# xvyaward/qeft

Measured on AMD Instinct MI355X. Metric: decode tokens/sec, Llama-2-7B w4 g128 r128, higher is better.
Workload: dtype f16; 1 GPU; llama-2-7b w4 g128 r128 full decode step, batch 1, greedy, KV context 69..1248 tokens (64-token context + 5 warm-up tokens before the timed region); layers=32, hipgraph=True, parallelism=single GPU

## Files before the change

### qeft_amd/csrc/decode_attn.h

```cpp
#pragma once
#include "qeft_common.h"

namespace qeft {

template <int CTRL>
__device__ __forceinline__ float dpp_mov(float v) {
    return __builtin_bit_cast(float, __builtin_amdgcn_update_dpp(0, __builtin_bit_cast(int, v), CTRL, 0xF, 0xF, true));
}
__device__ __forceinline__ float wave_max(float v) {
    v = fmaxf(v, dpp_mov<0xB1>(v));
    v = fmaxf(v, dpp_mov<0x4E>(v));
    v = fmaxf(v, dpp_mov<0x141>(v));
    v = fmaxf(v, dpp_mov<0x140>(v));
    v = fmaxf(v, __shfl_xor(v, 16));
    v = fmaxf(v, __shfl_xor(v, 32));
    return v;
}

__device__ __forceinline__ void st_agent(float* p, float v) { __hip_atomic_store(p, v, __ATOMIC_RELAXED, __HIP_MEMORY_SCOPE_AGENT); }
__device__ __forceinline__ float ld_agent(const float* p) { return __hip_atomic_load(p, __ATOMIC_RELAXED, __HIP_MEMORY_SCOPE_AGENT); }

constexpr int kAttnRec = 132;
__host__ __device__ constexpr size_t attn_ctr_floats(int n_heads) { return ((size_t)n_heads + 3) / 4 * 4; }

template <bool KFT>
__device__ __forceinline__ size_t kcache_off(int p, int chunk, int max_seq) {
    return KFT ? ((size_t)chunk * max_seq + p) * 8 : (size_t)p * 128 + chunk * 8;
}

template <int PRE, int DH = 1, bool KFT = false, bool DBG = false, bool ALIBI = false, bool ROW = true>
__device__ __forceinline__ void rope_attn_decode_body(uint8_t* smem_raw, const int bid, const int* __restrict__ pos_ptr,
                                                      const int* __restrict__ out_pos, const f16* __restrict__ q,
                                                      const f16* __restrict__ k, const f16* __restrict__ v,
                                                      const float* __restrict__ cs, uint32_t heads_kv_s_tab,
                                                      const float* __restrict__ sn, f16* __restrict__ kc, f16* __restrict__ vc,
                                                      f16* __restrict__ out, float* __restrict__ ws, int max_seq,
                                                      unsigned long long* dbg_ptr, const float* __restrict__ alibi,
                                                      f16* __restrict__ pub = nullptr) {
    constexpr int HD = 128;
    const int n_heads = (int)(heads_kv_s_tab & 0xfffu), n_kv = (int)((heads_kv_s_tab >> 12) & 0xfffu);
    const int S = (int)((heads_kv_s_tab >> 24) & 0xfu);
    unsigned long long* const dbg = DBG ? dbg_ptr : nullptr;
    unsigned long long stamp[10];
    auto mark = [&](int i) {
        if (dbg) { __builtin_amdgcn_sched_barrier(0); stamp[i] = __builtin_amdgcn_s_memtime(); __builtin_amdgcn_sched_barrier(0); }
    };
    unsigned long long rt0 = dbg ? __builtin_amdgcn_s_memrealtime() : 0;
    mark(0);
    float* prob = (float*)smem_raw;
    float* part = prob + max_seq + 16;
    float* psum = part + 16 * HD;
    float* wm = psum + 64;
    f16* knew = (f16*)(wm + 4);
    f16* vnew = knew + HD;
    f16* qs = vnew + HD;
    __shared__ int last_ticket;

    constexpr int HDB = HD / DH;
    constexpr int NDG = 16 / DH;
    constexpr int NPC = 64 / NDG;
    constexpr int PPC = 16 / NPC;
    const int dhi = (int)(bid % DH);
    const int hs_idx = bid / DH;
    const int h = hs_idx / S, sp = hs_idx % S, t = threadIdx.x, lane = t & 63;
    const int w = __builtin_amdgcn_readfirstlane(t >> 6);
    const int gw = sp * 4 + w, NW = 4 * S;
    const int grp = n_heads / n_kv, hk = h / grp;
    f16* kch = kc + (size_t)hk * max_seq * HD;
    f16* vch = vc + (size_t)hk * max_seq * HD;
    const bool appender = (sp == 0) && (dhi == 0) && (h % grp == 0);
    const float slope = ALIBI ? alibi[h] : 0.f;

    const int ti = dhi * HDB + (t & (HDB - 1));
    const f16* src = (t < 64) ? q + h * HD + t : (t < 128) ? k + hk * HD + (t - 64) : v + hk * HD + (t - 128);
    const f16 raw_a = src[0];
    const f16 raw_b = src[(t < 128) ? 64 : 0];
    float rc, rsn;
    if constexpr (ROW) {
        rc = cs[t & 63];
        rsn = sn[t & 63];
    }
    int opos_raw = 0;
    if (out_pos) opos_raw = out_pos[h * HD + ti];
    mark(1);
    const int pos = *pos_ptr, L = pos + 1;
    if (pos < 0 || pos >= max_seq) return;
    if (dbg) { asm volatile("" :: "s"(pos)); }
    if constexpr (!ROW) {
        rc = cs[(size_t)pos * 64 + (t & 63)];
        rsn = sn[(size_t)pos * 64 + (t & 63)];
    }
    mark(2);
    const int qd = lane & 3, pj = lane >> 2;
    const int dg = lane & (NDG - 1), pc = lane / NDG;
    const int dim0 = dhi * HDB + dg * 8;
    h8 kpre[PRE][4], vpre[PRE][PPC];
#pragma unroll
    for (int i = 0; i < PRE; ++i) {
        const int r0 = (i * NW + gw) * 16;
        const int krow = r0 < L ? r0 + pj : 0;
#pragma unroll
        for (int j = 0; j < 4; ++j) kpre[i][j] = *(const h8*)(kch + kcache_off<KFT>(krow, qd + 4 * j, max_seq));
    }
#pragma unroll
    for (int i = 0; i < PRE; ++i) {
        const int r0 = (i * NW + gw) * 16;
        const int vrow = r0 < L ? r0 + pc * PPC : 0;
        const h8* row = (const h8*)(vch + (size_t)vrow * HD + dim0);
#pragma unroll
        for (int j = 0; j < PPC; ++j) vpre[i][j] = row[j * (HD / 8)];
    }
    const int opos = out_pos ? opos_raw : h * HD + ti;
    const float ra = (float)raw_a, rb = (float)raw_b;
    const int i = t & 63;
    const float c = rc, sv = rsn;
    float r0 = ra * c - rb * sv, r1 = rb * c + ra * sv;
    asm("" : "+v"(r0), "+v"(r1));
    const float scale = 0.08838834764831845f;
    const f16 q0 = (f16)(r0 * scale), q1 = (f16)(r1 * scale);
    const f16 k0 = (f16)r0, k1 = (f16)r1;
    const f16 vv = (f16)ra;
    {
        f16* const d0 = knew + t + ((t < 64) ? 2 * HD : (t < 128) ? -64 : 0);
        d0[0] = (t < 64) ? q0 : (t < 128) ? k0 : vv;
        d0[(t < 128) ? 64 : 0] = (t < 64) ? q1 : (t < 128) ? k1 : vv;
    }
    if (appender) {
        if (t >= 128) {
            vch[(size_t)pos * HD + (t - 128)] = vv;
        } else if (t >= 64) {
            kch[kcache_off<KFT>(pos, i >> 3, max_seq) + (i & 7)] = k0;
            kch[kcache_off<KFT>(pos, (i >> 3) + 8, max_seq) + (i & 7)] = k1;
        }
    }
    asm volatile("s_waitcnt lgkmcnt(0)\n\ts_barrier" ::: "memory");
    mark(3);

    h2 qreg[16];
#pragma unroll
    for (int j = 0; j < 16; ++j) qreg[j] = *(const h2*)(qs + (j >> 2) * 32 + qd * 8 + 2 * (j & 3));
    float snew = 0.f;
#pragma unroll
    for (int j = 0; j < 16; ++j) snew = dot2(qreg[j], *(const h2*)(knew + (j >> 2) * 32 + qd * 8 + 2 * (j & 3)), snew);
    float lmax = -3.0e38f;
    auto score_run = [&](int i, const h8* kr, bool live) {
        const int p = (i * NW + gw) * 16 + pj;
        float sdot = 0.f;
#pragma unroll
        for (int j = 0; j < 4; ++j) {
            const u32x4 kw = __builtin_bit_cast(u32x4, kr[j]);
#pragma unroll
            for (int e = 0; e < 4; ++e) sdot = dot2(qreg[j * 4 + e], as_h2(kw[e]), sdot);
        }
        sdot = (p == pos) ? snew : sdot;
        sdot += dpp_mov<0xB1>(sdot);
        sdot += dpp_mov<0x4E>(sdot);
        if constexpr (ALIBI) sdot += slope * (float)(p - pos);
        sdot = (p >= L) ? -3.0e38f : sdot;
        if (qd == 0) prob[live ? p : max_seq + pj] = sdot;
        lmax = fmaxf(lmax, sdot);
    };
#pragma unroll
    for (int i = 0; i < PRE; ++i) score_run(i, kpre[i], (i * NW + gw) * 16 < L);
    for (int i = PRE; (i * NW + gw) * 16 < L; ++i) {
        h8 kr[4];
#pragma unroll
        for (int j = 0; j < 4; ++j) kr[j] = *(const h8*)(kch + kcache_off<KFT>((i * NW + gw) * 16 + pj, qd + 4 * j, max_seq));
        score_run(i, kr, true);
    }
    const float mw = wave_max(lmax);
    mark(4);
    __builtin_amdgcn_wave_barrier();

    float o[8];
#pragma unroll
    for (int e = 0; e < 8; ++e) o[e] = 0.f;
    float lsum = 0.f;
    const h8 vn = *(const h8*)(vnew + dim0);
    auto pv_run = [&](int i, const h8* vr, bool live) {
        const int p0 = (i * NW + gw) * 16 + pc * PPC;
        const int s0 = live ? p0 : max_seq + pc * PPC;
        float sraw[PPC];
#pragma unroll
        for (int j = 0; j < PPC; ++j) sraw[j] = prob[s0 + j];
#pragma unroll
        for (int j = 0; j < PPC; ++j) {
            const int p = p0 + j;
            const float ex = __expf(sraw[j] - mw);
            const float e = (p < L) ? ex : 0.f;
            const h8 vv = (p < pos) ? vr[j] : vn;
            lsum += e;
#pragma unroll
            for (int d = 0; d < 8; ++d) o[d] += e * (float)vv[d];
        }
    };
#pragma unroll
    for (int i = 0; i < PRE; ++i) pv_run(i, vpre[i], (i * NW + gw) * 16 < L);
    for (int i = PRE; (i * NW + gw) * 16 < L; ++i) {
        h8 vr[PPC];
#pragma unroll
        for (int j = 0; j < PPC; ++j)
            vr[j] = *(const h8*)(vch + (size_t)((i * NW + gw) * 16 + pc * PPC + j) * HD + dim0);
        pv_run(i, vr, true);
    }
    {
        float* dst = part + (w * NPC + pc) * HDB + dg * 8;
        *(f32x4*)dst = f32x4{o[0], o[1], o[2], o[3]};
        *(f32x4*)(dst + 4) = f32x4{o[4], o[5], o[6], o[7]};
        if (dg == 0) psum[w * NPC + pc] = lsum;
        if (lane == 0) wm[w] = mw;
    }
    mark(5);
    __syncthreads();
    mark(6);
    const float M = fmaxf(fmaxf(wm[0], wm[1]), fmaxf(wm[2], wm[3]));
    float acc = 0.f, den = 0.f;
    if (t < HDB) {
#pragma unroll
        for (int g = 0; g < 4 * NPC; ++g) {
            const float f = __expf(wm[g / NPC] - M);
            acc += f * part[g * HDB + t];
            den += f * psum[g];
        }
    }
    if (S == 1) {
        if (t < HDB) {
            const f16 ov = (f16)(acc / den);
            if (pub) __hip_atomic_store((uint16_t*)pub + opos, __builtin_bit_cast(uint16_t, ov), __ATOMIC_RELAXED, __HIP_MEMORY_SCOPE_AGENT);
            else out[opos] = ov;
        }
        if (dbg && lane == 0) {
            mark(7);
            unsigned long long* d = dbg + ((size_t)bid * 4 + w) * 12;
            d[0] = rt0; d[1] = __builtin_amdgcn_s_memrealtime();
            for (int i = 0; i < 8; ++i) d[2 + i] = stamp[i];
            d[10] = d[11] = 0;
        }
        return;
    }
    float* rec = ws + attn_ctr_floats(n_heads) + (size_t)(h * S + sp) * kAttnRec;
    if (t < HD) st_agent(rec + t, acc);
    if (t == 0) {
        st_agent(rec + HD, M);
        st_agent(rec + HD + 1, den);
    }
    asm volatile("s_waitcnt vmcnt(0)" ::: "memory");
    __syncthreads();
    mark(7);
    unsigned* ctr = (unsigned*)ws + h;
    if (t == 0) {
        const unsigned ticket = __hip_atomic_fetch_add(ctr, 1u, __ATOMIC_RELAXED, __HIP_MEMORY_SCOPE_AGENT);
        last_ticket = (ticket == (unsigned)(S - 1));
        if (ticket == (unsigned)(S - 1)) __hip_atomic_store(ctr, 0u, __ATOMIC_RELAXED, __HIP_MEMORY_SCOPE_AGENT);
    }
    __syncthreads();
    mark(8);
    if (dbg && lane == 0 && !last_ticket) {
        unsigned long long* d = dbg + ((size_t)bid * 4 + w) * 12;
        d[0] = rt0; d[1] = __builtin_amdgcn_s_memrealtime();
        for (int i = 0; i < 9; ++i) d[2 + i] = stamp[i];
        d[11] = 0;
    }
    if (!last_ticket) return;
    if (t < HD) {
        const float* r0 = ws + attn_ctr_floats(n_heads) + (size_t)h * S * kAttnRec;
        float Mh = -3.0e38f;
        for (int j = 0; j < S; ++j) Mh = fmaxf(Mh, ld_agent(r0 + j * kAttnRec + HD));
        float a2 = 0.f, d2 = 0.f;
        for (int j = 0; j < S; ++j) {
            const float f = __expf(ld_agent(r0 + j * kAttnRec + HD) - Mh);
            a2 += f * ld_agent(r0 + j * kAttnRec + t);
            d2 += f * ld_agent(r0 + j * kAttnRec + HD + 1);
        }
        out[opos] = (f16)(a2 / d2);
    }
    if (dbg && lane == 0) {
        mark(9);
        unsigned long long* d = dbg + ((size_t)bid * 4 + w) * 12;
        d[0] = rt0; d[1] = __builtin_amdgcn_s_memrealtime();
        for (int i = 0; i < 9; ++i) d[2 + i] = stamp[i];
        d[11] = stamp[9];
    }
}

template <int PRE, int DH = 1, bool KFT = false, bool DBG = false, bool ALIBI = false, bool ROW = true>
__global__ __launch_bounds__(256) void rope_attn_decode_kernel(const int* __restrict__ pos_ptr, const int* __restrict__ out_pos,
                                                               const f16* __restrict__ q, const f16* __restrict__ k,
                                                               const f16* __restrict__ v, const float* __restrict__ cs,
                                                               uint32_t heads_kv_s_tab, const float* __restrict__ sn,
                                                               f16* __restrict__ kc, f16* __restrict__ vc, f16* __restrict__ out,
                                                               float* __restrict__ ws, int max_seq, unsigned long long* dbg_ptr,
                                                               const float* __restrict__ alibi) {
    extern __shared__ __attribute__((aligned(16))) uint8_t smem_raw[];
    rope_attn_decode_body<PRE, DH, KFT, DBG, ALIBI, ROW>(smem_raw, (int)blockIdx.x, pos_ptr, out_pos, q, k, v, cs, heads_kv_s_tab, sn, kc, vc, out, ws,
                                                    max_seq, dbg_ptr, alibi);
}

__host__ __device__ inline size_t rope_attn_smem_bytes(int max_seq) { return (size_t)(max_seq + 16) * 4 + 16 * 128 * 4 + 64 * 4 + 4 * 4 + 3 * 128 * 2; }

}
```

### qeft_amd/csrc/decode_aux.hip

```cpp
#include <cstdlib>

#include "qeft_common.h"
#include "host_launch.h"
#include "decode_attn.h"

namespace qeft {

__device__ __forceinline__ float block_sum_256(float v, float* sm) {
    v = wave_sum(v);
    const int lane = threadIdx.x & 63, wave = threadIdx.x >> 6;
    __syncthreads();
    if (lane == 0) sm[wave] = v;
    __syncthreads();
    return sm[0] + sm[1] + sm[2] + sm[3];
}

__device__ __forceinline__ float block_max_256(float v, float* sm) {
#pragma unroll
    for (int o = 32; o > 0; o >>= 1) v = fmaxf(v, __shfl_xor(v, o));
    const int lane = threadIdx.x & 63, wave = threadIdx.x >> 6;
    __syncthreads();
    if (lane == 0) sm[wave] = v;
    __syncthreads();
    return fmaxf(fmaxf(sm[0], sm[1]), fmaxf(sm[2], sm[3]));
}

__global__ __launch_bounds__(256) void rmsnorm_kernel(const f16* __restrict__ x, const f16* __restrict__ add,
                                                      const f16* __restrict__ gamma, f16* __restrict__ res_out,
                                                      f16* __restrict__ y, int H, float eps) {
    __shared__ float sm[4];
    const size_t base = (size_t)blockIdx.x * H;
    float ss = 0.f;
    for (int i = threadIdx.x * 8; i < H; i += 256 * 8) {
        h8 v = *(const h8*)(x + base + i);
        if (add) {
            const h8 w = *(const h8*)(add + base + i);
#pragma unroll
            for (int j = 0; j < 8; ++j) v[j] = (f16)((float)v[j] + (float)w[j]);
            if (res_out) *(h8*)(res_out + base + i) = v;
        }
#pragma unroll
        for (int j = 0; j < 8; ++j) ss += (float)v[j] * (float)v[j];
    }
    ss = block_sum_256(ss, sm);
    const float rs = rsqrtf(ss / (float)H + eps);
    for (int i = threadIdx.x * 8; i < H; i += 256 * 8) {
        h8 v = *(const h8*)(x + base + i);
        if (add) {
            const h8 w = *(const h8*)(add + base + i);
#pragma unroll
            for (int j = 0; j < 8; ++j) v[j] = (f16)((float)v[j] + (float)w[j]);
        }
        const h8 g = *(const h8*)(gamma + i);
        h8 o;
#pragma unroll
        for (int j = 0; j < 8; ++j) o[j] = mul_f32_to_f16((float)v[j] * rs, (float)g[j]);
        *(h8*)(y + base + i) = o;
    }
}

__global__ __launch_bounds__(256) void silu_mul_kernel(const f16* __restrict__ gate, const f16* __restrict__ up,
                                                       f16* __restrict__ out, int n) {
    const int i = (blockIdx.x * 256 + threadIdx.x) * 8;
    if (i >= n) return;
    const h8 g = *(const h8*)(gate + i), u = *(const h8*)(up + i);
    h8 o;
#pragma unroll
    for (int j = 0; j < 8; ++j) {
        o[j] = mul_f32_to_f16(silu_f32((float)g[j]), (float)u[j]);
    }
    *(h8*)(out + i) = o;
}

__global__ __launch_bounds__(256) void token_begin_kernel(const f16* __restrict__ embed, const long long* __restrict__ tok,
                                                          const float* __restrict__ rope_tab, const int* __restrict__ pos,
                                                          f16* __restrict__ h, float* __restrict__ rope_row, int hidden,
                                                          int vocab, int max_seq) {
    const long long tk = min(max(*tok, 0ll), (long long)vocab - 1);
    const int i = (blockIdx.x * 256 + threadIdx.x) * 8;
    if (i < hidden) *(h8*)(h + i) = *(const h8*)(embed + (size_t)tk * hidden + i);
    if (blockIdx.x == 0 && threadIdx.x < 128 && rope_row) {
        const int p = min(max(*pos, 0), max_seq - 1);
        rope_row[threadIdx.x] = rope_tab[(size_t)p * 128 + threadIdx.x];
    }
}

__global__ __launch_bounds__(256) void token_begin_norm_kernel(const f16* __restrict__ embed, const long long* __restrict__ tok,
                                                               const float* __restrict__ rope_tab, const int* __restrict__ pos,
                                                               float* __restrict__ h, float* __restrict__ rope_row,
                                                               const f16* __restrict__ gamma, f16* __restrict__ hnorm,
                                                               float* __restrict__ ssq_out, int hidden, int vocab, int max_seq) {
    __shared__ float sm[4];
    const long long tk = min(max(*tok, 0ll), (long long)vocab - 1);
    const int i = (blockIdx.x * 256 + threadIdx.x) * 8;
    float ss = 0.f;
    if (i < hidden) {
        const h8 v = *(const h8*)(embed + (size_t)tk * hidden + i), g = *(const h8*)(gamma + i);
        h8 o;
#pragma unroll
        for (int j = 0; j < 8; ++j) {
            ss += (float)v[j] * (float)v[j];
            o[j] = mul_f32_to_f16((float)v[j], (float)g[j]);
            h[i + j] = (float)v[j];
        }
        *(h8*)(hnorm + i) = o;
    }
    ss = block_sum_256(ss, sm);
    if (threadIdx.x == 0) ssq_out[blockIdx.x] = ss;
    if (blockIdx.x == 0 && threadIdx.x < 128 && rope_row) {
        const int p = min(max(*pos, 0), max_seq - 1);
        rope_row[threadIdx.x] = rope_tab[(size_t)p * 128 + threadIdx.x];
    }
}

__global__ __launch_bounds__(256) void residual_norm_kernel(const float* __restrict__ h, const f16* __restrict__ add,
                                                            const f16* __restrict__ gamma, float* __restrict__ h_out,
                                                            f16* __restrict__ hnorm, float* __restrict__ ssq_out, int hidden) {
    __shared__ float sm[4];
    const int i = (blockIdx.x * 256 + threadIdx.x) * 8;
    float ss = 0.f;
    if (i < hidden) {
        float v[8];
#pragma unroll
        for (int j = 0; j < 8; ++j) v[j] = h[i + j];
        if (add) {
            const h8 w = *(const h8*)(add + i);
#pragma unroll
            for (int j = 0; j < 8; ++j) v[j] += (float)w[j];
        }
#pragma unroll
        for (int j = 0; j < 8; ++j) h_out[i + j] = v[j];
        if (gamma) {
            const h8 g = *(const h8*)(gamma + i);
            h8 o;
#pragma unroll
            for (int j = 0; j < 8; ++j) {
                ss += v[j] * v[j];
                o[j] = mul_f32_to_f16(v[j], (float)g[j]);
            }
            *(h8*)(hnorm + i) = o;
        }
    }
    if (gamma) {
        ss = block_sum_256(ss, sm);
        if (threadIdx.x == 0) ssq_out[blockIdx.x] = ss;
    }
}

__global__ __launch_bounds__(256) void rmsnorm_f32_kernel(const float* __restrict__ x, const f16* __restrict__ gamma,
                                                          f16* __restrict__ y, int H, float eps) {
    __shared__ float sm[4];
    const size_t base = (size_t)blockIdx.x * H;
    float ss = 0.f;
    for (int i = threadIdx.x; i < H; i += 256) ss += x[base + i] * x[base + i];
    ss = block_sum_256(ss, sm);
    const float rs = rsqrtf(ss / (float)H + eps);
    for (int i = threadIdx.x; i < H; i += 256) y[base + i] = mul_f32_to_f16(x[base + i] * rs, (float)gamma[i]);
}

__global__ __launch_bounds__(256) void rope_rows_kernel(f16* __restrict__ x, const float* __restrict__ cs,
                                                        const float* __restrict__ sn, int H, int row_stride) {
    const int t = blockIdx.x, i = threadIdx.x & 63;
    const float c = cs[(size_t)t * 64 + i], s = sn[(size_t)t * 64 + i];
    for (int h = threadIdx.x >> 6; h < H; h += 4) {
        f16* p = x + (size_t)t * row_stride + h * 128;
        const float a = (float)p[i], b = (float)p[i + 64];
        p[i] = (f16)(a * c - b * s);
        p[i + 64] = (f16)(b * c + a * s);
    }
}

hipError_t rope_rows_launch(void* x, const void* cs, const void* sn, int T, int H, int row_stride, hipStream_t st) {
    hipLaunchKernelGGL(rope_rows_kernel, dim3(T), dim3(256), 0, st, (f16*)x, (const float*)cs, (const float*)sn, H, row_stride);
    return hipGetLastError();
}

template <int LPR>
__global__ __launch_bounds__(512) void lm_head_f16_kernel(const float* __restrict__ h32, const f16* __restrict__ gamma,
                                                          const f16* __restrict__ W, f16* __restrict__ logits, int vocab,
                                                          float eps, int rows_per_block) {
    constexpr int H = 512 * LPR;
    __shared__ float red[8];
    const int tid = threadIdx.x, lane = tid & 63;
    const int wave = __builtin_amdgcn_readfirstlane(tid >> 6);
    float xv[LPR][8];
    float ss = 0.f;
#pragma unroll
    for (int c = 0; c < LPR; ++c) {
        const f32x4 a = *(const f32x4*)(h32 + c * 512 + lane * 8), b = *(const f32x4*)(h32 + c * 512 + lane * 8 + 4);
#pragma unroll
        for (int j = 0; j < 4; ++j) {
            xv[c][j] = a[j];
            xv[c][4 + j] = b[j];
            ss += a[j] * a[j] + b[j] * b[j];
        }
    }
    ss = wave_sum(ss);
    const float rs = rsqrtf(ss / (float)H + eps);
    h2 xh[LPR][4];
#pragma unroll
    for (int c = 0; c < LPR; ++c) {
        const h8 g = *(const h8*)(gamma + c * 512 + lane * 8);
#pragma unroll
        for (int j = 0; j < 4; ++j)
            xh[c][j] = h2{mul_f32_to_f16(xv[c][2 * j] * rs, (float)g[2 * j]), mul_f32_to_f16(xv[c][2 * j + 1] * rs, (float)g[2 * j + 1])};
    }
    (void)red;
    const int r_end = min(vocab, (int)(blockIdx.x + 1) * rows_per_block);
    int r = blockIdx.x * rows_per_block + wave;
    u32x4 cur[LPR], nxt[LPR];
    auto load_row = [&](int row, u32x4 (&dst)[LPR]) {
        const u32x4* p = (const u32x4*)(W + (size_t)min(row, vocab - 1) * H) + lane;
#pragma unroll
        for (int c = 0; c < LPR; ++c) dst[c] = __builtin_nontemporal_load(p + c * 64);
    };
    load_row(r, cur);
    for (; r < r_end; r += 8) {
        load_row(r + 8, nxt);
        float acc = 0.f;
#pragma unroll
        for (int c = 0; c < LPR; ++c)
#pragma unroll
            for (int j = 0; j < 4; ++j) acc = __builtin_amdgcn_fdot2(as_h2(cur[c][j]), xh[c][j], acc, false);
        acc = wave_sum(acc);
        if (lane == 0) logits[r] = (f16)acc;
#pragma unroll
        for (int c = 0; c < LPR; ++c) cur[c] = nxt[c];
    }
}

hipError_t lm_head_f16_launch(const void* h32, const void* gamma, const void* W, void* logits, int H, int vocab, float eps,
                              hipStream_t st) {
    const int blocks = vocab >= 4096 ? 512 : (vocab + 7) / 8, rpb = (vocab + blocks - 1) / blocks;
    auto go = [&](auto kern) {
        hipLaunchKernelGGL(kern, dim3(blocks), dim3(512), 0, st, (const float*)h32, (const f16*)gamma, (const f16*)W, (f16*)logits,
                           vocab, eps, rpb);
        return hipGetLastError();
    };
    switch (H) {
        case 512: return go(lm_head_f16_kernel<1>);
        case 1024: return go(lm_head_f16_kernel<2>);
        case 2048: return go(lm_head_f16_kernel<4>);
        case 4096: return go(lm_head_f16_kernel<8>);
        case 5120: return go(lm_head_f16_kernel<10>);
        case 8192: return go(lm_head_f16_kernel<16>);
        default: return hipErrorInvalidValue;
    }
}

__global__ __launch_bounds__(1024) void token_end_kernel(const f16* __restrict__ logits, long long* __restrict__ tok,
                                                         int* __restrict__ pos, int vocab, int greedy) {
    __shared__ float bv[16];
    __shared__ int bi[16];
    const int t = threadIdx.x;
    if (greedy) {
        float best = -INFINITY;
        int idx = 0x7fffffff;
        for (int i = t * 8; i < vocab; i += 1024 * 8) {
            if (i + 8 <= vocab) {
                const h8 v = *(const h8*)(logits + i);
#pragma unroll
                for (int j = 0; j < 8; ++j)
                    if ((float)v[j] > best) { best = (float)v[j]; idx = i + j; }
            } else {
                for (int j = i; j < vocab; ++j)
                    if ((float)logits[j] > best) { best = (float)logits[j]; idx = j; }
            }
        }
#pragma unroll
        for (int o = 32; o > 0; o >>= 1) {
            const float ob = __shfl_xor(best, o);
            const int oi = __shfl_xor(idx, o);
            if (ob > best || (ob == best && oi < idx)) { best = ob; idx = oi; }
        }
        if ((t & 63) == 0) { bv[t >> 6] = best; bi[t >> 6] = idx; }
        __syncthreads();
        if (t == 0) {
            for (int w = 1; w < 16; ++w)
                if (bv[w] > best || (bv[w] == best && bi[w] < idx)) { best = bv[w]; idx = bi[w]; }
            *tok = idx == 0x7fffffff ? 0 : idx;
        }
    }
    if (t == 0) *pos = *pos + 1;
}

hipError_t token_begin_launch(const void* embed, const void* tok, const void* rope_tab, const int* pos, void* h,
                              void* rope_row, int hidden, int vocab, int max_seq, hipStream_t st) {
    hipLaunchKernelGGL(token_begin_kernel, dim3((hidden / 8 + 255) / 256), dim3(256), 0, st, (const f16*)embed,
                       (const long long*)tok, (const float*)rope_tab, pos, (f16*)h, (float*)rope_row, hidden, vocab, max_seq);
    return hipGetLastError();
}

int token_begin_norm_blocks(int hidden) { return (hidden / 8 + 255) / 256; }

hipError_t token_begin_norm_launch(const void* embed, const void* tok, const void* rope_tab, const int* pos, void* h,
                                   void* rope_row, const void* gamma, void* hnorm, float* ssq_out, int hidden, int vocab,
                                   int max_seq, hipStream_t st) {
    hipLaunchKernelGGL(token_begin_norm_kernel, dim3(token_begin_norm_blocks(hidden)), dim3(256), 0, st, (const f16*)embed,
                       (const long long*)tok, (const float*)rope_tab, pos, (float*)h, (float*)rope_row, (const f16*)gamma,
                       (f16*)hnorm, ssq_out, hidden, vocab, max_seq);
    return hipGetLastError();
}

hipError_t residual_norm_launch(const void* h, const void* add, const void* gamma, void* h_out, void* hnorm, float* ssq_out,
                                int hidden, hipStream_t st) {
    hipLaunchKernelGGL(residual_norm_kernel, dim3(token_begin_norm_blocks(hidden)), dim3(256), 0, st, (const float*)h,
                       (const f16*)add, (const f16*)gamma, (float*)h_out, (f16*)hnorm, ssq_out, hidden);
    return hipGetLastError();
}

hipError_t rmsnorm_f32_launch(const void* x, const void* gamma, void* y, int m, int H, float eps, hipStream_t st) {
    hipLaunchKernelGGL(rmsnorm_f32_kernel, dim3(m), dim3(256), 0, st, (const float*)x, (const f16*)gamma, (f16*)y, H, eps);
    return hipGetLastError();
}

hipError_t token_end_launch(const void* logits, void* tok, int* pos, int vocab, int greedy, hipStream_t st) {
    hipLaunchKernelGGL(token_end_kernel, dim3(1), dim3(1024), 0, st, (const f16*)logits, (long long*)tok, pos, vocab, greedy);
    return hipGetLastError();
}

hipError_t rmsnorm_launch(const void* x, const void* add, const void* gamma, void* res_out, void* y, int m, int H,
                          float eps, hipStream_t st) {
    hipLaunchKernelGGL(rmsnorm_kernel, dim3(m), dim3(256), 0, st, (const f16*)x, (const f16*)add, (const f16*)gamma,
                       (f16*)res_out, (f16*)y, H, eps);
    return hipGetLastError();
}

hipError_t silu_mul_launch(const void* gate, const void* up, void* out, int n, hipStream_t st) {
    hipLaunchKernelGGL(silu_mul_kernel, dim3((n / 8 + 255) / 256), dim3(256), 0, st, (const f16*)gate, (const f16*)up,
                       (f16*)out, n);
    return hipGetLastError();
}

unsigned long long* g_attn_dbg = nullptr;
#ifndef QEFT_ATTN_PRE1
#define QEFT_ATTN_PRE1 4
#endif
size_t attn_workspace_bytes(int n_heads, int S) { return S > 1 ? (attn_ctr_floats(n_heads) + (size_t)n_heads * S * kAttnRec) * 4 : 0; }

hipError_t rope_attn_decode_launch(const void* q, const void* k, const void* v, const void* cs, const void* sn, void* kc,
                                   void* vc, const int* pos, const int* out_pos, void* out, void* ws, int n_heads,
                                   int n_kv, int max_seq, int S, int tab_rows, hipStream_t st, bool k_ft_layout,
                                   const float* alibi_slopes) {
    const size_t smem = (size_t)(max_seq + 16) * 4 + 16 * 128 * 4 + 64 * 4 + 4 * 4 + 3 * 128 * 2;
    int dh = 1;
    auto launch = [&](auto kern) -> hipError_t {
        if (smem > 64 * 1024) {
            hipError_t e = hipFuncSetAttribute((const void*)kern, hipFuncAttributeMaxDynamicSharedMemorySize, (int)smem);
            if (e != hipSuccess) return e;
        }
        if (n_heads > 4095 || n_kv > 4095 || S > 15) return hipErrorInvalidValue;
        const uint32_t packed = (uint32_t)n_heads | ((uint32_t)n_kv << 12) | ((uint32_t)S << 24);
        hipLaunchKernelGGL(kern, dim3(n_heads * S * dh), dim3(256), smem, st, pos, out_pos, (const f16*)q, (const f16*)k,
                           (const f16*)v, (const float*)cs, packed, (const float*)sn, (f16*)kc, (f16*)vc, (f16*)out, (float*)ws,
                           max_seq, g_attn_dbg, alibi_slopes);
        return hipGetLastError();
    };
    static const int dh_env = getenv("QEFT_ATTN_DH") ? atoi(getenv("QEFT_ATTN_DH")) : 2;
    const bool row = tab_rows == 1;
#define QEFT_ATTN_FORM(...) (row ? launch(rope_attn_decode_kernel<__VA_ARGS__, true>) : launch(rope_attn_decode_kernel<__VA_ARGS__, false>))
    if (k_ft_layout) {
        if (S != 1) return hipErrorInvalidValue;
        if (alibi_slopes) return QEFT_ATTN_FORM(4, 1, true, false, true);
        return QEFT_ATTN_FORM(4, 1, true, false, false);
    }
    if (g_attn_dbg) {
        if (S == 1 && dh_env == 2) {
            dh = 2;
            return QEFT_ATTN_FORM(4, 2, false, true, false);
        }
        if (S == 1) return QEFT_ATTN_FORM(4, 1, false, true, false);
        if (S == 2) return QEFT_ATTN_FORM(2, 1, false, true, false);
        return QEFT_ATTN_FORM(1, 1, false, true, false);
    }
    if (S == 1 && dh_env == 4) {
        dh = 4;
        return QEFT_ATTN_FORM(QEFT_ATTN_PRE1, 4, false, false, false);
    }
    if (S == 1 && dh_env == 2) {
        dh = 2;
        return QEFT_ATTN_FORM(QEFT_ATTN_PRE1, 2, false, false, false);
    }
    if (S == 1) return QEFT_ATTN_FORM(QEFT_ATTN_PRE1, 1, false, false, false);
    if (S == 2) return QEFT_ATTN_FORM(2, 1, false, false, false);
    return QEFT_ATTN_FORM(1, 1, false, false, false);
#undef QEFT_ATTN_FORM
}

__global__ __launch_bounds__(256) void sqa_generic_kernel(const f16* __restrict__ q, const f16* __restrict__ k, const f16* __restrict__ v,
                                                          f16* __restrict__ kc, f16* __restrict__ vc, const int* __restrict__ pos_ptr,
                                                          const float* __restrict__ alibi, f16* __restrict__ out, int n_heads, int n_kv,
                                                          int max_seq, int D) {
    extern __shared__ __attribute__((aligned(16))) uint8_t smem_raw[];
    float* qs = (float*)smem_raw;
    float* knew = qs + 256;
    float* vnew = knew + 256;
    float* red = vnew + 256;
    float* prob = red + 256;
    const int h = blockIdx.x, t = threadIdx.x;
    const int grp = n_heads / n_kv, hk = h / grp;
    const int pos = *pos_ptr, L = pos + 1;
    if (pos < 0 || pos >= max_seq) return;
    f16* kch = kc + (size_t)hk * max_seq * D;
    f16* vch = vc + (size_t)hk * max_seq * D;
    const float scale = __builtin_amdgcn_rsqf((float)D);
    if (t < D) {
        const f16 kv = k[hk * D + t], vv = v[hk * D + t];
        qs[t] = (float)q[h * D + t] * scale;
        knew[t] = (float)kv;
        vnew[t] = (float)vv;
        if (h % grp == 0) {
            kch[((size_t)(t >> 3) * max_seq + pos) * 8 + (t & 7)] = kv;
            vch[(size_t)pos * D + t] = vv;
        }
    }
    __syncthreads();
    const float slope = alibi ? alibi[h] : 0.f;
    float lmax = -3.0e38f;
    for (int p = t; p < L; p += 256) {
        float sdot = 0.f;
        if (p == pos) {
            for (int d = 0; d < D; ++d) sdot += qs[d] * knew[d];
        } else {
            for (int c = 0; c < D / 8; ++c) {
                const h8 kk = *(const h8*)(kch + ((size_t)c * max_seq + p) * 8);
#pragma unroll
                for (int e = 0; e < 8; ++e) sdot += qs[c * 8 + e] * (float)kk[e];
            }
        }
        sdot += slope * (float)(p - pos);
        prob[p] = sdot;
        lmax = fmaxf(lmax, sdot);
    }
    red[t] = lmax;
    __syncthreads();
    for (int s = 128; s > 0; s >>= 1) {
        if (t < s) red[t] = fmaxf(red[t], red[t + s]);
        __syncthreads();
    }
    const float m = red[0];
    __syncthreads();
    float lsum = 0.f;
    for (int p = t; p < L; p += 256) {
        const float e = __expf(prob[p] - m);
        prob[p] = e;
        lsum += e;
    }
    red[t] = lsum;
    __syncthreads();
    for (int s = 128; s > 0; s >>= 1) {
        if (t < s) red[t] += red[t + s];
        __syncthreads();
    }
    const float inv = 1.f / red[0];
    __syncthreads();
    const int NG = 256 / D > 0 ? 256 / D : 1;
    float o = 0.f;
    const int d = t % D, pcl = t / D;
    if (pcl < NG)
        for (int p = pcl; p < L; p += NG) o += prob[p] * (p == pos ? vnew[d] : (float)vch[(size_t)p * D + d]);
    red[t] = pcl < NG ? o : 0.f;
    __syncthreads();
    if (t < D) {
        float acc = 0.f;
        for (int g = 0; g < NG; ++g) acc += red[g * D + t];
        out[h * D + t] = (f16)(acc * inv);
    }
}

hipError_t sqa_generic_launch(const void* q, const void* k, const void* v, void* kc, void* vc, const int* pos, const float* alibi,
                              void* out, int n_heads, int n_kv, int max_seq, int head_dim, hipStream_t st) {
    const size_t smem = (size_t)(4 * 256 + max_seq) * 4;
    if (smem > 64 * 1024) {
        const hipError_t e = hipFuncSetAttribute((const void*)sqa_generic_kernel, hipFuncAttributeMaxDynamicSharedMemorySize, (int)smem);
        if (e != hipSuccess) return e;
    }
    hipLaunchKernelGGL(sqa_generic_kernel, dim3(n_heads), dim3(256), smem, st, (const f16*)q, (const f16*)k, (const f16*)v, (f16*)kc, (f16*)vc,
                       pos, alibi, (f16*)out, n_heads, n_kv, max_seq, head_dim);
    return hipGetLastError();
}

}
```

Measured before the change: 766.8 tokens/s.

## Prefetch early KV cache rows before reading decode position in attention

Issues the first EARLY K (and possibly V) cache loads before the dependent load of the position pointer, so the cache fetches overlap that load instead of waiting behind it. The rows loaded early are bounded by max_seq rather than the live length. Kernel arguments are repacked into a geometry word with a power-of-two group shift, log2 of the split count and max_seq/16, which replaces integer divisions. A new table form reads sin from the cos table when the two are contiguous. The early loads may fetch rows beyond the live context, costing some extra bandwidth, and the split count is now limited to powers of two up to 8.

```diff
diff --git a/qeft_amd/csrc/decode_attn.h b/qeft_amd/csrc/decode_attn.h
--- a/qeft_amd/csrc/decode_attn.h
+++ b/qeft_amd/csrc/decode_attn.h
@@ -28,18 +28,20 @@
     return KFT ? ((size_t)chunk * max_seq + p) * 8 : (size_t)p * 128 + chunk * 8;
 }
 
-template <int PRE, int DH = 1, bool KFT = false, bool DBG = false, bool ALIBI = false, bool ROW = true>
-__device__ __forceinline__ void rope_attn_decode_body(uint8_t* smem_raw, const int bid, const int* __restrict__ pos_ptr,
-                                                      const int* __restrict__ out_pos, const f16* __restrict__ q,
+template <int PRE, int DH = 1, bool KFT = false, bool DBG = false, bool ALIBI = false, int ROW = 1, int EARLY_ = 0>
+__device__ __forceinline__ void rope_attn_decode_body(uint8_t* smem_raw, const int bid, const f16* __restrict__ q,
                                                       const f16* __restrict__ k, const f16* __restrict__ v,
-                                                      const float* __restrict__ cs, uint32_t heads_kv_s_tab,
-                                                      const float* __restrict__ sn, f16* __restrict__ kc, f16* __restrict__ vc,
-                                                      f16* __restrict__ out, float* __restrict__ ws, int max_seq,
+                                                      const float* __restrict__ cs, const int* __restrict__ out_pos,
+                                                      f16* __restrict__ kc, uint32_t geom, int n_heads, f16* __restrict__ vc,
+                                                      const float* __restrict__ sn, const int* __restrict__ pos_ptr,
+                                                      f16* __restrict__ out, float* __restrict__ ws,
                                                       unsigned long long* dbg_ptr, const float* __restrict__ alibi,
                                                       f16* __restrict__ pub = nullptr) {
     constexpr int HD = 128;
-    const int n_heads = (int)(heads_kv_s_tab & 0xfffu), n_kv = (int)((heads_kv_s_tab >> 12) & 0xfffu);
-    const int S = (int)((heads_kv_s_tab >> 24) & 0xfu);
+    constexpr int EARLY = ROW == 0 ? 0 : EARLY_ < PRE ? EARLY_ : PRE;
+    const int grp = (int)(geom & 0xfffu), gsh = (int)((geom >> 12) & 0xfu);
+    const int lgS = DH > 1 ? 0 : (int)((geom >> 16) & 3u), S = 1 << lgS;
+    const int max_seq = (int)((geom >> 18) & 0xfffu) * 16;
     unsigned long long* const dbg = DBG ? dbg_ptr : nullptr;
     unsigned long long stamp[10];
     auto mark = [&](int i) {
@@ -60,15 +62,14 @@
     constexpr int NDG = 16 / DH;
     constexpr int NPC = 64 / NDG;
     constexpr int PPC = 16 / NPC;
-    const int dhi = (int)(bid % DH);
-    const int hs_idx = bid / DH;
-    const int h = hs_idx / S, sp = hs_idx % S, t = threadIdx.x, lane = t & 63;
+    const int dhi = (int)((unsigned)bid % DH);
+    const int hs_idx = (int)((unsigned)bid / DH);
+    const int h = hs_idx >> lgS, sp = hs_idx & (S - 1), t = threadIdx.x, lane = t & 63;
     const int w = __builtin_amdgcn_readfirstlane(t >> 6);
     const int gw = sp * 4 + w, NW = 4 * S;
-    const int grp = n_heads / n_kv, hk = h / grp;
+    const int hk = gsh ? h >> (gsh - 1) : h / grp;
     f16* kch = kc + (size_t)hk * max_seq * HD;
-    f16* vch = vc + (size_t)hk * max_seq * HD;
-    const bool appender = (sp == 0) && (dhi == 0) && (h % grp == 0);
+    const bool appender = (sp == 0) && (dhi == 0) && (h == hk * grp);
     const float slope = ALIBI ? alibi[h] : 0.f;
 
     const int ti = dhi * HDB + (t & (HDB - 1));
@@ -76,39 +77,63 @@
     const f16 raw_a = src[0];
     const f16 raw_b = src[(t < 128) ? 64 : 0];
     float rc, rsn;
-    if constexpr (ROW) {
+    if constexpr (ROW != 0) {
         rc = cs[t & 63];
-        rsn = sn[t & 63];
+        rsn = ROW == 2 ? cs[64 + (t & 63)] : sn[t & 63];
     }
     int opos_raw = 0;
     if (out_pos) opos_raw = out_pos[h * HD + ti];
-    mark(1);
-    const int pos = *pos_ptr, L = pos + 1;
-    if (pos < 0 || pos >= max_seq) return;
-    if (dbg) { asm volatile("" :: "s"(pos)); }
-    if constexpr (!ROW) {
-        rc = cs[(size_t)pos * 64 + (t & 63)];
-        rsn = sn[(size_t)pos * 64 + (t & 63)];
-    }
-    mark(2);
     const int qd = lane & 3, pj = lane >> 2;
     const int dg = lane & (NDG - 1), pc = lane / NDG;
     const int dim0 = dhi * HDB + dg * 8;
     h8 kpre[PRE][4], vpre[PRE][PPC];
-#pragma unroll
-    for (int i = 0; i < PRE; ++i) {
+    auto k_run = [&](int i, int krow) {
+#pragma unroll
+        for (int j = 0; j < 4; ++j) kpre[i][j] = *(const h8*)(kch + kcache_off<KFT>(krow, qd + 4 * j, max_seq));
+    };
+    f16* vch;
+    auto v_run = [&](int i, int vrow) {
+        const h8* row = (const h8*)(vch + (size_t)vrow * HD + dim0);
+#pragma unroll
+        for (int j = 0; j < PPC; ++j) vpre[i][j] = row[j * (HD / 8)];
+    };
+    auto early_r0 = [&](int i) {
         const int r0 = (i * NW + gw) * 16;
-        const int krow = r0 < L ? r0 + pj : 0;
-#pragma unroll
-        for (int j = 0; j < 4; ++j) kpre[i][j] = *(const h8*)(kch + kcache_off<KFT>(krow, qd + 4 * j, max_seq));
-    }
-#pragma unroll
-    for (int i = 0; i < PRE; ++i) {
+        return r0 < max_seq ? r0 : 0;
+    };
+#pragma unroll
+    for (int i = 0; i < EARLY; ++i) k_run(i, early_r0(i) + pj);
+    if constexpr (EARLY > 0) __builtin_amdgcn_sched_barrier(0);
+    vch = vc + (size_t)hk * max_seq * HD;
+    if constexpr (EARLY > 0) asm volatile("" ::"s"(vch));
+    if constexpr (EARLY == PRE) {
+#pragma unroll
+        for (int i = 0; i < EARLY; ++i) v_run(i, early_r0(i) + pc * PPC);
+    }
+    mark(1);
+    int pos_raw = -1;
+    if (EARLY == 0 || pos_ptr) pos_raw = *pos_ptr;
+    const int pos = pos_raw, L = pos + 1;
+    if (pos < 0 || pos >= max_seq) return;
+    if (dbg) { asm volatile("" :: "s"(pos)); }
+    if constexpr (ROW == 0) {
+        rc = cs[(size_t)pos * 64 + (t & 63)];
+        rsn = sn[(size_t)pos * 64 + (t & 63)];
+    }
+    mark(2);
+#pragma unroll
+    for (int i = EARLY; i < PRE; ++i) {
         const int r0 = (i * NW + gw) * 16;
-        const int vrow = r0 < L ? r0 + pc * PPC : 0;
-        const h8* row = (const h8*)(vch + (size_t)vrow * HD + dim0);
-#pragma unroll
-        for (int j = 0; j < PPC; ++j) vpre[i][j] = row[j * (HD / 8)];
+        k_run(i, r0 < L ? r0 + pj : 0);
+    }
+    if constexpr (EARLY < PRE) {
+#pragma unroll
+        for (int i = 0; i < EARLY; ++i) v_run(i, early_r0(i) + pc * PPC);
+    }
+#pragma unroll
+    for (int i = EARLY; i < PRE; ++i) {
+        const int r0 = (i * NW + gw) * 16;
+        v_run(i, r0 < L ? r0 + pc * PPC : 0);
     }
     const int opos = out_pos ? opos_raw : h * HD + ti;
     const float ra = (float)raw_a, rb = (float)raw_b;
@@ -283,17 +308,27 @@
     }
 }
 
-template <int PRE, int DH = 1, bool KFT = false, bool DBG = false, bool ALIBI = false, bool ROW = true>
-__global__ __launch_bounds__(256) void rope_attn_decode_kernel(const int* __restrict__ pos_ptr, const int* __restrict__ out_pos,
-                                                               const f16* __restrict__ q, const f16* __restrict__ k,
+template <int PRE, int DH = 1, bool KFT = false, bool DBG = false, bool ALIBI = false, int ROW = 1, int EARLY = 0>
+__global__ __launch_bounds__(256) void rope_attn_decode_kernel(const f16* __restrict__ q, const f16* __restrict__ k,
                                                                const f16* __restrict__ v, const float* __restrict__ cs,
-                                                               uint32_t heads_kv_s_tab, const float* __restrict__ sn,
-                                                               f16* __restrict__ kc, f16* __restrict__ vc, f16* __restrict__ out,
-                                                               float* __restrict__ ws, int max_seq, unsigned long long* dbg_ptr,
+                                                               const int* __restrict__ out_pos, f16* __restrict__ kc, uint32_t geom,
+                                                               int n_heads, f16* __restrict__ vc, const float* __restrict__ sn,
+                                                               const int* __restrict__ pos_ptr, f16* __restrict__ out,
+                                                               float* __restrict__ ws, unsigned long long* dbg_ptr,
                                                                const float* __restrict__ alibi) {
     extern __shared__ __attribute__((aligned(16))) uint8_t smem_raw[];
-    rope_attn_decode_body<PRE, DH, KFT, DBG, ALIBI, ROW>(smem_raw, (int)blockIdx.x, pos_ptr, out_pos, q, k, v, cs, heads_kv_s_tab, sn, kc, vc, out, ws,
-                                                    max_seq, dbg_ptr, alibi);
+    rope_attn_decode_body<PRE, DH, KFT, DBG, ALIBI, ROW, EARLY>(smem_raw, (int)blockIdx.x, q, k, v, cs, out_pos, kc, geom, n_heads, vc, sn,
+                                                                pos_ptr, out, ws, dbg_ptr, alibi);
+}
+
+inline uint32_t rope_attn_geom(int n_heads, int n_kv, int S, int max_seq) {
+    const int grp = n_kv > 0 ? n_heads / n_kv : 0;
+    if (grp < 1 || grp > 4095 || (S != 1 && S != 2 && S != 4 && S != 8) || max_seq < 16 || max_seq % 16 || max_seq > 32768) return 0;
+    uint32_t gsh = 0, lgS = 0;
+    if ((grp & (grp - 1)) == 0)
+        while ((1 << gsh++) != grp) {}
+    while ((1 << lgS) != S) ++lgS;
+    return (uint32_t)grp | (gsh << 12) | (lgS << 16) | ((uint32_t)(max_seq / 16) << 18);
 }
 
 __host__ __device__ inline size_t rope_attn_smem_bytes(int max_seq) { return (size_t)(max_seq + 16) * 4 + 16 * 128 * 4 + 64 * 4 + 4 * 4 + 3 * 128 * 2; }
diff --git a/qeft_amd/csrc/decode_aux.hip b/qeft_amd/csrc/decode_aux.hip
--- a/qeft_amd/csrc/decode_aux.hip
+++ b/qeft_amd/csrc/decode_aux.hip
@@ -336,29 +336,35 @@
 #ifndef QEFT_ATTN_PRE1
 #define QEFT_ATTN_PRE1 4
 #endif
+#ifndef QEFT_ATTN_EARLY
+#define QEFT_ATTN_EARLY 2
+#endif
 size_t attn_workspace_bytes(int n_heads, int S) { return S > 1 ? (attn_ctr_floats(n_heads) + (size_t)n_heads * S * kAttnRec) * 4 : 0; }
 
 hipError_t rope_attn_decode_launch(const void* q, const void* k, const void* v, const void* cs, const void* sn, void* kc,
                                    void* vc, const int* pos, const int* out_pos, void* out, void* ws, int n_heads,
                                    int n_kv, int max_seq, int S, int tab_rows, hipStream_t st, bool k_ft_layout,
                                    const float* alibi_slopes) {
-    const size_t smem = (size_t)(max_seq + 16) * 4 + 16 * 128 * 4 + 64 * 4 + 4 * 4 + 3 * 128 * 2;
+    const size_t smem = rope_attn_smem_bytes(max_seq);
     int dh = 1;
     auto launch = [&](auto kern) -> hipError_t {
         if (smem > 64 * 1024) {
             hipError_t e = hipFuncSetAttribute((const void*)kern, hipFuncAttributeMaxDynamicSharedMemorySize, (int)smem);
             if (e != hipSuccess) return e;
         }
-        if (n_heads > 4095 || n_kv > 4095 || S > 15) return hipErrorInvalidValue;
-        const uint32_t packed = (uint32_t)n_heads | ((uint32_t)n_kv << 12) | ((uint32_t)S << 24);
-        hipLaunchKernelGGL(kern, dim3(n_heads * S * dh), dim3(256), smem, st, pos, out_pos, (const f16*)q, (const f16*)k,
-                           (const f16*)v, (const float*)cs, packed, (const float*)sn, (f16*)kc, (f16*)vc, (f16*)out, (float*)ws,
-                           max_seq, g_attn_dbg, alibi_slopes);
+        const uint32_t geom = rope_attn_geom(n_heads, n_kv, S, max_seq);
+        if (n_heads > 4095 || !geom || (dh > 1 && S != 1)) return hipErrorInvalidValue;
+        hipLaunchKernelGGL(kern, dim3(n_heads * S * dh), dim3(256), smem, st, (const f16*)q, (const f16*)k, (const f16*)v,
+                           (const float*)cs, out_pos, (f16*)kc, geom, n_heads, (f16*)vc, (const float*)sn, pos, (f16*)out,
+                           (float*)ws, g_attn_dbg, alibi_slopes);
         return hipGetLastError();
     };
     static const int dh_env = getenv("QEFT_ATTN_DH") ? atoi(getenv("QEFT_ATTN_DH")) : 2;
-    const bool row = tab_rows == 1;
-#define QEFT_ATTN_FORM(...) (row ? launch(rope_attn_decode_kernel<__VA_ARGS__, true>) : launch(rope_attn_decode_kernel<__VA_ARGS__, false>))
+    const int form = tab_rows != 1 ? 0 : (const float*)sn == (const float*)cs + 64 ? 2 : 1;
+#define QEFT_ATTN_FORM(...)                                                          \
+    (form == 2   ? launch(rope_attn_decode_kernel<__VA_ARGS__, 2, QEFT_ATTN_EARLY>)  \
+     : form == 1 ? launch(rope_attn_decode_kernel<__VA_ARGS__, 1, QEFT_ATTN_EARLY>)  \
+                 : launch(rope_attn_decode_kernel<__VA_ARGS__, 0, QEFT_ATTN_EARLY>))
     if (k_ft_layout) {
         if (S != 1) return hipErrorInvalidValue;
         if (alibi_slopes) return QEFT_ATTN_FORM(4, 1, true, false, true);
```

Result: faster. 776.6 tokens/s, median of 6 (+1.3%).
